# xander683/ConstructionScenePoseEstimation

Hardware: AMD Instinct MI355X
Metric: annotated frames/sec (RGB+seg+2D kpts) at 1920×1080, 1/2/4/8 MI355X (higher is better)
Workload: dtype f32

## Files before the change

constructionsceneposeestimation_amd/build.py:

```python
from __future__ import annotations

import os
import shutil
import subprocess
import sys

PKG = os.path.dirname(os.path.abspath(__file__))
ROOT = os.path.dirname(PKG)
LIB = os.path.join(PKG, "libcsg.so")
SOURCES = [os.path.join(PKG, "csrc", "csg_kernels.hip"), os.path.join(PKG, "csrc", "csg_encode.hip"),
           os.path.join(PKG, "csrc", "csg_crops.hip"), os.path.join(PKG, "csrc", "csg_spans.hip"),
           os.path.join(PKG, "csrc", "csg_amodal_spans.hip"), os.path.join(PKG, "csrc", "csg_api.cpp")]
DEPS = SOURCES + [os.path.join(PKG, "csrc", "csg_kernels.h"), os.path.join(PKG, "csrc", "csg_encode.h"),
                  os.path.join(PKG, "csrc", "csg_deflate.h"), os.path.join(PKG, "csrc", "csg_widen.h"),
                  os.path.join(PKG, "csrc", "csg_crops.h"), os.path.join(PKG, "csrc", "csg_spans.h"),
                  os.path.join(PKG, "csrc", "csg_amodal_spans.h"), os.path.join(PKG, "csrc", "csg_raster_math.h"),
                  os.path.join(PKG, "csrc", "csg_amodal_tri.inc"),
                  os.path.join(ROOT, "include", "csg_api.h")]
ARCH = os.environ.get("CSG_OFFLOAD_ARCH", "gfx950")
IO_LIB = os.path.join(PKG, "libcsgio.so")
IO_SOURCES = [os.path.join(PKG, "csrc", "csg_io.cpp")]
IO_DEPS = IO_SOURCES + [os.path.join(ROOT, "include", "csg_io.h"), os.path.join(PKG, "csrc", "csg_repr.h")]
IO_FLAGS = ["-O3", "-std=c++17", "-fPIC", "-shared", "-Wall", "-pthread"]
JSON_EXT = os.path.join(PKG, "_csgjson.so")
JSON_SOURCES = [os.path.join(PKG, "csrc", "csg_json.cpp"), os.path.join(PKG, "csrc", "csg_repr.h")]

FLAGS = ["-O3", "-std=c++17", "-fPIC", "-shared", "-ffp-contract=off", f"--offload-arch={ARCH}", "-Wall", "-pthread"]


def hipcc() -> str:
    for c in (os.environ.get("HIPCC"), "/opt/rocm/bin/hipcc", shutil.which("hipcc")):
        if c and os.path.exists(c):
            return c
    raise RuntimeError("hipcc not found (ROCm required to build libcsg.so)")


def needs_build(lib: str = LIB, deps=None) -> bool:
    deps = DEPS if deps is None else deps
    if not os.path.exists(lib):
        return True
    t = os.path.getmtime(lib)
    return any(os.path.getmtime(p) > t for p in deps)


def build(force: bool = False, verbose: bool = False) -> str:
    if force or needs_build():
        cmd = [hipcc(), *FLAGS, "-o", LIB + ".tmp", *SOURCES]
        if verbose:
            print(" ".join(cmd), file=sys.stderr)
        subprocess.run(cmd, check=True)
# ... 33 lines not shown
```

constructionsceneposeestimation_amd/csrc/csg_api.cpp:

```cpp
#include <hip/hip_runtime.h>
#include <stdint.h>
#include <stdlib.h>
#include <string.h>

#include <algorithm>
#include <cstddef>
#include <cmath>
#include <cstdarg>
#include <cstdio>
#include <memory>
#include <string>
#include <vector>

#include "../../include/csg_api.h"
#include "csg_amodal_spans.h"
#include "csg_crops.h"
#include "csg_encode.h"
#include "csg_kernels.h"
#include "csg_spans.h"
#include "csg_widen.h"

using namespace csg;

namespace {

template <class T>
struct DevBuf {
  T* p = nullptr;
  size_t n = 0;
  DevBuf() = default;
  DevBuf(const DevBuf&) = delete;
  DevBuf& operator=(const DevBuf&) = delete;
  ~DevBuf() { release(); }
  hipError_t alloc(size_t count) {
    if (count <= n && p) return hipSuccess;
    if (p) (void)hipFree(p);
    p = nullptr;
    n = 0;
    if (count == 0) return hipSuccess;
    hipError_t e = hipMalloc(reinterpret_cast<void**>(&p), count * sizeof(T));
    if (e == hipSuccess) n = count;
    return e;
  }
  void release() {
    if (p) (void)hipFree(p);
    p = nullptr;
    n = 0;
  }
};

constexpr uint32_t kAutoChainFrames = 0xFFFFFFFFu;

constexpr uint32_t kMaxSets = 65536;

struct HostTexture {
  std::vector<uint8_t> rgba;
  uint32_t w = 0, h = 0;
  bool present = false;
};

}

struct csg_ctx {
  csg_config cfg{};
  std::string err;
  hipStream_t stream = nullptr;
  uint32_t tiles_x = 0, tiles_y = 0, n_tiles = 0;

  bool have_scene = false;
  uint32_t n_inst = 0, n_meshes = 0, n_materials = 0;
  uint64_t n_tris_total = 0;
  DevBuf<float> tri_pos, tri_uv;
  DevBuf<InstDesc> inst;
  std::vector<MatDesc> h_mats;
  std::vector<MatDesc> h_set_mats;
  std::vector<MeshDesc> h_meshes;
  DevBuf<Chunk> chunks;
  uint32_t n_chunks = 0;
  uint32_t uid_shift = kUidShift;
  std::vector<HostTexture> textures;
  bool tex_dirty = true;
  DevBuf<uint8_t> texels;
  DevBuf<uint32_t> aquad;
  DevBuf<uint32_t> acls;
  std::vector<int> acls_thr;
  DevBuf<TexDesc> texd;
  LightDev light{{0.26f, 0.29f, 0.34f}, {0.78f, 0.78f, 0.78f}, {0.7071f, 0.f, 0.7071f},
                 191u | (217u << 8) | (255u << 16)};
  std::vector<LightDev> dr_light;
  std::vector<uint8_t> dr_light_valid;
  std::vector<int32_t> dr_tex;
  bool dr_dirty = true;
  DevBuf<LightDev> lights;
  DevBuf<MatDesc> set_mats;
  uint32_t n_table_sets = 0;
  std::vector<float> h_models;
  std::vector<uint8_t> set_valid;
  DevBuf<float> models;
  bool models_dirty = true;
  uint32_t n_kp = 0;
  std::vector<float> h_kp;
  std::vector<uint8_t> kp_valid;
  DevBuf<float> kp;
  bool kp_dirty = true;
  uint32_t n_lab = 1;
// ... 158 lines not shown
    const double g = (x >= 1.0 / 8 && x < 3.0 / 8) ? 4 * x - 0.5 : (x >= 3.0 / 8 && x < 5.0 / 8) ? 1.0
                     : (x >= 5.0 / 8 && x < 7.0 / 8) ? -4 * x + 3.5 : 0.0;
    const double b = (x < 1.0 / 8) ? 4 * x + 0.5 : (x >= 1.0 / 8 && x < 3.0 / 8) ? 1.0
                     : (x >= 3.0 / 8 && x < 5.0 / 8) ? -4 * x + 2.5 : 0.0;
    const double ch[3] = {r, g, b};
    uint32_t v = 0;
    for (int c = 0; c < 3; ++c) {
      const float p = (float)ch[c] * 255.0f;
      const long q = std::lrint(p);
      v |= (uint32_t)std::min(255L, std::max(0L, q)) << (8 * c);
    }
    lut[k] = v;
  }
}

extern "C" {

int csg_abi_version(void) { return CSG_ABI_VERSION; }

const char* csg_last_error(const csg_ctx* ctx) { return ctx ? ctx->err.c_str() : "null context"; }

int csg_create(const csg_config* cfg, csg_ctx** out) {
  if (!cfg || !out) return CSG_ERR_INVALID;
  *out = nullptr;
  if (cfg->width == 0 || cfg->height == 0 || cfg->width > 256u * kTileW || cfg->height > 512u * kTileH ||
      cfg->max_frames == 0 ||
      !(cfg->near_clip >= 0x1p-126f) || !(cfg->far_clip > cfg->near_clip) || !(cfg->far_clip <= 0x1p126f))
    return CSG_ERR_INVALID;
  csg_ctx* c = new csg_ctx();
  c->cfg = *cfg;
  if (const char* d = getenv("CSG_DEBUG")) c->dbg = (uint32_t)strtoul(d, nullptr, 0);
  if (const char* v = getenv("CSG_NARROW_IDS")) c->narrow_ids = atoi(v) != 0;
  if (const char* v = getenv("CSG_SPLIT_PAGEABLE")) c->split_pageable = atoi(v) != 0;
  c->chain_frames = cfg->frames_per_launch ? cfg->frames_per_launch : kAutoChainFrames;
  if (const char* v = getenv("CSG_CHAIN")) c->chain_frames = (uint32_t)std::max(1, atoi(v));
  c->chain_frames = std::min(c->chain_frames, cfg->max_frames);
  c->tiles_x = (cfg->width + kTileW - 1) / kTileW;
  c->tiles_y = (cfg->height + kTileH - 1) / kTileH;
  c->n_tiles = c->tiles_x * c->tiles_y;
  c->bin_blocks = kTileH >= 32 ? 32u : (c->n_tiles > 8192u ? 8u : 16u);
  if (const char* v = getenv("CSG_BINBLOCKS")) c->bin_blocks = std::max(1, std::min(1024, atoi(v)));
  hipError_t e = hipSetDevice(cfg->device);
  if (e == hipSuccess) e = hipStreamCreateWithFlags(&c->stream, hipStreamNonBlocking);
  c->ring.assign((size_t)csg_ctx::kRing * 5, nullptr);
  c->ring_frames.assign(csg_ctx::kRing, 0);
  for (size_t k = 0; k < c->ring.size() && e == hipSuccess; ++k) e = hipEventCreate(&c->ring[k]);
  for (uint32_t k = 0; k < csg_ctx::kStaging && e == hipSuccess; ++k)
    e = hipEventCreateWithFlags(&c->stage_ev[k], hipEventDisableTiming);
  if (e == hipSuccess) e = c->overflow.alloc(16);
  if (e == hipSuccess) e = hipMemset(c->overflow.p, 0, 16 * sizeof(uint32_t));
  if (e == hipSuccess) e = c->jet.alloc(256);
  if (e == hipSuccess) {
    uint32_t lut[256];
    jet_lut(lut);
    e = hipMemcpy(c->jet.p, lut, sizeof(lut), hipMemcpyHostToDevice);
  }
  c->ev = c->ring.data();
  if (e != hipSuccess) {
    c->err = hipGetErrorString(e);
    csg_destroy(c);
    return CSG_ERR_DEVICE;
  }
  *out = c;
  return CSG_OK;
}

void csg_destroy(csg_ctx* c) {
  if (!c) return;
  if (c->last_stream && c->last_stream != c->stream) (void)hipStreamSynchronize(c->last_stream);
  if (c->stream) (void)hipStreamSynchronize(c->stream);
  if (c->copy_stream) (void)hipStreamSynchronize(c->copy_stream);
  c->tri_pos.release(); c->tri_uv.release(); c->inst.release(); c->set_mats.release(); c->iset.release(); c->lights.release();
  c->chunks.release();
  c->texels.release();
  c->aquad.release();
  c->acls.release();
  c->texd.release(); c->models.release(); c->kp.release(); c->frames.release(); c->clip.release();
  c->pv.release(); c->recs.release(); c->rect.release(); c->rec_count.release(); c->tile_count.release();
  c->slab.release(); c->plan_need.release();
  c->tile_off.release(); c->bins.release(); c->bcount.release(); c->overflow.release(); c->o_rgb.release();
  c->o_inst.release(); c->o_depth.release(); c->o_kp_uv.release(); c->o_kp_vis.release(); c->o_stats.release();
  c->kp_w.release(); c->kp_pix.release(); c->kp_tiles.release();
  c->o_points.release(); c->o_normals.release(); c->cam.release(); c->fset.release();
  c->of.release(); c->o_objc.release();
  c->o_dvis.release(); c->o_drange.release(); c->o_cov.release(); c->drange.release(); c->jet.release();
  for (uint32_t k = 0; k < csg_ctx::kStaging; ++k) {
    if (c->h_stage[k]) (void)hipHostFree(c->h_stage[k]);
    if (c->stage_ev[k]) (void)hipEventDestroy(c->stage_ev[k]);
  }
  if (c->am_busy) (void)hipEventSynchronize(c->am_done);
  c->lab_off.release(); c->lab_chunks.release(); c->am_frames.release(); c->am_bits.release(); c->am_keys.release();
  for (uint32_t k = 0; k < csg_ctx::kStaging; ++k) {
    if (c->am_stage[k]) (void)hipHostFree(c->am_stage[k]);
    if (c->am_stage_ev[k]) (void)hipEventDestroy(c->am_stage_ev[k]);
  }
  c->as_planes.release(); c->as_touched.release(); c->as_cnt.release(); c->as_tables.release();
  if (c->as_stage) (void)hipHostFree(c->as_stage);
  if (c->as_stage_ev) (void)hipEventDestroy(c->as_stage_ev);
  if (c->am_done) (void)hipEventDestroy(c->am_done);
  if (c->ms_busy) (void)hipEventSynchronize(c->ms_done);
  c->ms_cnt.release();
  if (c->ms_done) (void)hipEventDestroy(c->ms_done);
  for (auto& e : c->ring)
    if (e) (void)hipEventDestroy(e);
  if (c->h_ids_n) (void)hipHostFree(c->h_ids_n);
// ... 108 lines not shown
  HIP_TRY(c, c->chunks.alloc(ch.size()));
  HIP_TRY(c, hipMemcpy(c->tri_pos.p, tri_pos.data(), tri_pos.size() * 4, hipMemcpyHostToDevice));
  HIP_TRY(c, hipMemcpy(c->tri_uv.p, tri_uv.data(), tri_uv.size() * 4, hipMemcpyHostToDevice));
  HIP_TRY(c, hipMemcpy(c->inst.p, idesc.data(), idesc.size() * sizeof(InstDesc), hipMemcpyHostToDevice));
  c->h_inst = idesc;
  {
    int32_t lo = -1, hi = -1;
    for (const InstDesc& d : idesc) { lo = std::min(lo, d.label); hi = std::max(hi, d.label); }
    c->ids_bytes = lo < -1 ? 4u : hi <= 254 ? 1u : hi <= 65534 ? 2u : 4u;
    c->n_lab = (uint32_t)std::max<int64_t>((int64_t)hi + 1, 1);
  }
  {
    std::vector<uint32_t> off((size_t)c->n_lab + 1, 0u), list;
    for (const Chunk& k : ch)
      if (idesc[k.inst].label >= 0) ++off[(size_t)idesc[k.inst].label + 1];
    uint32_t most = 0;
    for (uint32_t l = 0; l < c->n_lab; ++l) {
      most = std::max(most, off[l + 1]);
      off[l + 1] += off[l];
    }
    list.resize(std::max<size_t>(off[c->n_lab], 1), 0u);
    std::vector<uint32_t> at(off.begin(), off.end() - 1);
    for (size_t k = 0; k < ch.size(); ++k)
      if (idesc[ch[k].inst].label >= 0) list[at[(size_t)idesc[ch[k].inst].label]++] = (uint32_t)k;
    HIP_TRY(c, c->lab_off.alloc(off.size()));
    HIP_TRY(c, c->lab_chunks.alloc(list.size()));
    HIP_TRY(c, hipMemcpy(c->lab_off.p, off.data(), off.size() * 4, hipMemcpyHostToDevice));
    HIP_TRY(c, hipMemcpy(c->lab_chunks.p, list.data(), list.size() * 4, hipMemcpyHostToDevice));
    c->lab_max_chunks = most;
    c->h_lab_off = off;
    c->h_lab_chunks = list;
  }
  c->iset.release();
  HIP_TRY(c, hipMemcpy(c->chunks.p, ch.data(), ch.size() * sizeof(Chunk), hipMemcpyHostToDevice));
  c->n_inst = n_inst;
  c->n_meshes = n_meshes;
  c->n_materials = n_materials;
  c->h_mats = mats;
  c->h_meshes = md;
  c->n_chunks = (uint32_t)ch.size();
  c->n_tris_total = ntot;
  c->h_models = models;
  c->set_valid.assign(1, 1);
  c->models_dirty = true;
  c->dr_tex.clear();
  c->dr_dirty = true;
  c->h_kp.clear();
  c->kp_valid.clear();
  c->n_kp = 0;
  c->kp_dirty = true;
  c->h_of.clear();
  c->of_sets = 0;
  c->of_dirty = true;
  c->have_scene = true;
  c->work_frames = 0;
  c->rec_cap = 0;
  c->bin_cap = 0;
  return CSG_OK;
}

int csg_upload_texture(csg_ctx* c, uint32_t tex_id, const uint8_t* rgba8, uint32_t w, uint32_t h) {
  if (!c) return CSG_ERR_INVALID;
  if (!rgba8 || w == 0 || h == 0 || w > 16384 || h > 16384 || tex_id >= 4096)
    return c->fail(CSG_ERR_INVALID, "upload_texture: bad arguments");
  if (c->textures.size() <= tex_id) c->textures.resize(tex_id + 1);
  HostTexture& t = c->textures[tex_id];
// ... 104 lines not shown

static int build_alpha_classes(csg_ctx* c, const std::vector<TexDesc>& td, size_t total, bool tex_changed) {
  std::vector<int> thr(c->textures.size(), -1);
  for (const MatDesc& m : c->h_set_mats) {
    if (!m.alpha_test || m.texture < 0 || (size_t)m.texture >= thr.size()) continue;
    int& t = thr[m.texture];
    if (t == -1) t = (int)m.alpha_threshold;
    else if (t != (int)m.alpha_threshold) t = -2;
  }
  if (!tex_changed && c->acls.p && thr == c->acls_thr) return CSG_OK;
  c->acls_thr = thr;
  std::vector<uint32_t> cls((total + 15) / 16 + 1, 0xFFFFFFFFu);
  for (size_t k = 0; k < c->textures.size(); ++k) {
    const HostTexture& t = c->textures[k];
    if (!t.present || thr[k] < 0) continue;
    const uint32_t th = (uint32_t)thr[k];
    for (uint32_t y = 0; y < t.h; ++y)
      for (uint32_t x = 0; x < t.w; ++x) {
        const uint32_t x1 = x + 1 == t.w ? 0 : x + 1, y1 = y + 1 == t.h ? 0 : y + 1;
        auto a = [&](uint32_t xx, uint32_t yy) { return (uint32_t)t.rgba[((size_t)yy * t.w + xx) * 4 + 3]; };
        const uint32_t q[4] = {a(x, y), a(x1, y), a(x, y1), a(x1, y1)};
        const uint32_t mn = std::min(std::min(q[0], q[1]), std::min(q[2], q[3]));
        const uint32_t mx = std::max(std::max(q[0], q[1]), std::max(q[2], q[3]));
        const uint32_t cl = mx <= th ? 0u : mn > th ? 1u : 3u;
        const size_t i = (size_t)td[k].offset + (size_t)y * t.w + x;
        cls[i >> 4] = (cls[i >> 4] & ~(3u << (2 * (i & 15)))) | (cl << (2 * (i & 15)));
      }
  }
  HIP_TRY(c, c->acls.alloc(cls.size()));
  HIP_TRY(c, hipMemcpy(c->acls.p, cls.data(), cls.size() * 4, hipMemcpyHostToDevice));
  return CSG_OK;
}

static int sync_scene_state(csg_ctx* c) {
  const uint32_t n_sets = (uint32_t)c->set_valid.size();
  if (c->tex_dirty || c->dr_dirty || c->models_dirty || (c->kp_dirty && c->n_kp) || c->n_table_sets != n_sets) {
    const int rc = drain(c);
    if (rc) return rc;
    if (c->am_busy) HIP_TRY(c, hipEventSynchronize(c->am_done));
  }
  const bool tex_changed = c->tex_dirty;
  const bool iset_dirty = c->tex_dirty || c->dr_dirty || c->n_table_sets != n_sets || !c->iset.p;
  const bool cls_dirty = c->tex_dirty || c->dr_dirty || c->n_table_sets != n_sets || !c->acls.p;
  std::vector<TexDesc> td(c->textures.size());
  size_t total = 0;
  for (size_t k = 0; k < c->textures.size(); ++k) {
    td[k] = TexDesc{(uint32_t)total, c->textures[k].w, c->textures[k].h, 0};
    total += ((size_t)c->textures[k].w * c->textures[k].h + kTexAlign - 1) / kTexAlign * kTexAlign;
  }
  if (total / kTexAlign >= 0xFFFFFFu)
    return c->fail(CSG_ERR_LIMIT, "textures hold %zu texels; at most %u", total, 0xFFFFFFu * kTexAlign);
  if (c->tex_dirty) {
    HIP_TRY(c, c->texels.alloc(std::max<size_t>(total * 4, 4)));
    HIP_TRY(c, c->aquad.alloc(std::max<size_t>(total, 1)));
    HIP_TRY(c, c->texd.alloc(std::max<size_t>(td.size(), 1)));
    std::vector<uint32_t> quad;
    for (size_t k = 0; k < c->textures.size(); ++k)
      if (c->textures[k].present) {
        const HostTexture& t = c->textures[k];
        HIP_TRY(c, hipMemcpy(c->texels.p + (size_t)td[k].offset * 4, t.rgba.data(), t.rgba.size(),
                             hipMemcpyHostToDevice));
        quad.resize((size_t)t.w * t.h);
        for (uint32_t y = 0; y < t.h; ++y)
          for (uint32_t x = 0; x < t.w; ++x) {
            const uint32_t x1 = x + 1 == t.w ? 0 : x + 1, y1 = y + 1 == t.h ? 0 : y + 1;
            auto a = [&](uint32_t xx, uint32_t yy) { return (uint32_t)t.rgba[((size_t)yy * t.w + xx) * 4 + 3]; };
            quad[(size_t)y * t.w + x] = a(x, y) | (a(x1, y) << 8) | (a(x, y1) << 16) | (a(x1, y1) << 24);
          }
        HIP_TRY(c, hipMemcpy(c->aquad.p + td[k].offset, quad.data(), quad.size() * 4, hipMemcpyHostToDevice));
      }
    if (!td.empty()) HIP_TRY(c, hipMemcpy(c->texd.p, td.data(), td.size() * sizeof(TexDesc), hipMemcpyHostToDevice));
    c->tex_dirty = false;
  }
  if (c->dr_dirty || c->n_table_sets != n_sets) {
    std::vector<MatDesc> sm((size_t)n_sets * c->n_materials);
    std::vector<LightDev> sl(n_sets);
    for (uint32_t set = 0; set < n_sets; ++set) {
      sl[set] = (set < c->dr_light_valid.size() && c->dr_light_valid[set]) ? c->dr_light[set] : c->light;
      for (uint32_t m = 0; m < c->n_materials; ++m) {
        MatDesc d = c->h_mats[m];
        const size_t k = (size_t)set * c->n_materials + m;
        if (k < c->dr_tex.size() && c->dr_tex[k] != CSG_KEEP_TEXTURE) d.texture = c->dr_tex[k];
        sm[(size_t)set * c->n_materials + m] = d;
      }
    }
    HIP_TRY(c, c->set_mats.alloc(std::max<size_t>(sm.size(), 1)));
    HIP_TRY(c, c->lights.alloc(std::max<size_t>(sl.size(), 1)));
    c->h_set_mats = sm;
    if (!sm.empty()) HIP_TRY(c, hipMemcpy(c->set_mats.p, sm.data(), sm.size() * sizeof(MatDesc), hipMemcpyHostToDevice));
    if (!sl.empty()) HIP_TRY(c, hipMemcpy(c->lights.p, sl.data(), sl.size() * sizeof(LightDev), hipMemcpyHostToDevice));
    c->n_table_sets = n_sets;
    c->dr_dirty = false;
  }
  if (cls_dirty) {
    const int rc = build_alpha_classes(c, td, total, tex_changed);
    if (rc) return rc;
  }
  for (size_t k = 0; k < c->h_set_mats.size(); ++k) {
    const int t = c->h_set_mats[k].texture;
    if (t >= 0 && ((size_t)t >= c->textures.size() || !c->textures[t].present))
      return c->fail(CSG_ERR_INVALID, "material %u (set %u) references texture %d that was not uploaded",
                     (unsigned)(k % c->n_materials), (unsigned)(k / c->n_materials), t);
  }
  if (iset_dirty) {
    std::vector<InstSetDev> is((size_t)n_sets * c->n_inst);
    for (uint32_t set = 0; set < n_sets; ++set)
      for (uint32_t i = 0; i < c->n_inst; ++i) {
        const InstDesc& d = c->h_inst[i];
        const MatDesc& m = c->h_set_mats[(size_t)set * c->n_materials + d.material];
        InstSetDev e{};
        e.tex = (m.texture >= 0 && d.has_uv) ? m.texture : -1;
        e.base = (uint32_t)m.base[0] | ((uint32_t)m.base[1] << 8) | ((uint32_t)m.base[2] << 16);
        e.atex = kNoAlpha;
        if (m.alpha_test && m.texture >= 0) {
          const TexDesc& t = td[(size_t)m.texture];
          e.atex = t.offset;
          e.atex_wh = t.width | (t.height << 16);
          e.athr = m.alpha_threshold;
        }
        e.label = d.label;
        e.alpha_uv = (m.alpha_test && d.has_uv) ? 1u : 0u;
        is[(size_t)set * c->n_inst + i] = e;
      }
    HIP_TRY(c, c->iset.alloc(std::max<size_t>(is.size(), 1)));
    if (!is.empty()) HIP_TRY(c, hipMemcpy(c->iset.p, is.data(), is.size() * sizeof(InstSetDev), hipMemcpyHostToDevice));
  }
  if (c->models_dirty) {
    HIP_TRY(c, c->models.alloc(c->h_models.size()));
    HIP_TRY(c, hipMemcpy(c->models.p, c->h_models.data(), c->h_models.size() * 4, hipMemcpyHostToDevice));
    c->models_dirty = false;
  }
  if (c->kp_dirty && c->n_kp) {
    HIP_TRY(c, c->kp.alloc(c->h_kp.size()));
    HIP_TRY(c, hipMemcpy(c->kp.p, c->h_kp.data(), c->h_kp.size() * 4, hipMemcpyHostToDevice));
    c->kp_dirty = false;
  }
  return CSG_OK;
}

static int sync_object_frames(csg_ctx* c) {
  const uint32_t n_sets = (uint32_t)c->set_valid.size();
  if (!c->of_dirty && c->of_table_sets == n_sets && c->of.p) return CSG_OK;
  const int rc = drain(c);
  if (rc) return rc;
  if (c->am_busy) HIP_TRY(c, hipEventSynchronize(c->am_done));
  const size_t per = (size_t)c->n_lab * 12;
  std::vector<float> t((size_t)n_sets * per, 0.f);
  const size_t have = std::min<size_t>(c->of_sets, n_sets) * per;
  if (have) memcpy(t.data(), c->h_of.data(), have * sizeof(float));
  HIP_TRY(c, c->of.alloc(std::max<size_t>(t.size(), 12)));
  if (!t.empty()) HIP_TRY(c, hipMemcpy(c->of.p, t.data(), t.size() * 4, hipMemcpyHostToDevice));
  c->of_table_sets = n_sets;
  c->of_dirty = false;
  return CSG_OK;
// ... 48 lines not shown
                                       : (uint32_t)std::min<uint64_t>(3ull * c->rec_cap + 16ull * c->n_tiles,
                                                                      0x7FFFFFFCull);
  uint64_t rp, bp;
  target_pools(c, maxF, rp, bp);
  if (rp != c->rec_pool || bp != c->bin_pool) {
    c->recs.release(); c->rect.release(); c->bins.release();
  }
  HIP_TRY(c, c->frames.alloc(c->cfg.max_frames));
  for (uint32_t k = 0; k < csg_ctx::kStaging; ++k)
    if (!c->h_stage[k])
      HIP_TRY(c, hipHostMalloc(reinterpret_cast<void**>(&c->h_stage[k]), sizeof(FrameDev) * c->cfg.max_frames));
  HIP_TRY(c, c->fset.alloc(maxF));
  HIP_TRY(c, c->clip.alloc((size_t)maxF * c->n_inst * 12));
  HIP_TRY(c, c->pv.alloc((size_t)maxF * 12));
  HIP_TRY(c, c->cam.alloc((size_t)maxF * kCamFloats));
  c->rec_pool = c->bin_pool = 0;
  HIP_TRY(c, c->recs.alloc(rp));
  HIP_TRY(c, c->rect.alloc(rp));
  HIP_TRY(c, c->bins.alloc(bp));
  c->rec_pool = rp;
  c->bin_pool = bp;
  HIP_TRY(c, c->rec_count.alloc((size_t)maxF * kCounterStride));
  HIP_TRY(c, c->tile_count.alloc((size_t)maxF * c->n_tiles));
  HIP_TRY(c, c->tile_off.alloc((size_t)maxF * (c->n_tiles + 1)));
  HIP_TRY(c, c->bcount.alloc((size_t)maxF * c->bin_blocks * c->n_tiles));
  HIP_TRY(c, c->slab.alloc(maxF));
  HIP_TRY(c, c->plan_need.alloc(2));
  c->work_frames = maxF;
  return CSG_OK;
}

static SceneDev scene_dev(const csg_ctx* c) {
  SceneDev s{};
  s.tri_pos = c->tri_pos.p; s.tri_uv = c->tri_uv.p; s.inst = c->inst.p;
  s.texd = c->texd.p; s.texels = c->texels.p; s.aquad = c->aquad.p; s.acls = c->acls.p; s.n_inst = c->n_inst;
  s.W = c->cfg.width; s.H = c->cfg.height;
  s.tiles_x = c->tiles_x; s.tiles_y = c->tiles_y; s.n_tiles = c->n_tiles;
  s.near_clip = c->cfg.near_clip; s.far_clip = c->cfg.far_clip;
  s.inv_near = 1.0f / c->cfg.near_clip; s.inv_far = 1.0f / c->cfg.far_clip;
  s.dbg = c->dbg;
  s.uid_shift = c->uid_shift;
  s.rect_ys = c->tiles_y > 256u ? 1u : 0u;
  return s;
}

static bool host_pinned(const void* p) {
  hipPointerAttribute_t a{};
  if (hipPointerGetAttributes(&a, p) != hipSuccess) {
    (void)hipGetLastError();
    return false;
  }
  return a.type == hipMemoryTypeHost;
}

struct WidenChain {
  const void* src;
  uint32_t bytes;
  int32_t* dst;
  size_t n;
  std::shared_ptr<WidenLatch> latch;
};
static void widen_submit_cb(void* p) {
  std::unique_ptr<WidenChain> w(static_cast<WidenChain*>(p));
  WidenPool::get().submit(w->src, w->bytes, w->dst, w->n, w->latch);
}
static void widen_wait_cb(void* p) {
  std::unique_ptr<std::shared_ptr<WidenLatch>> l(static_cast<std::shared_ptr<WidenLatch>*>(p));
// ... 1310 lines not shown
```

constructionsceneposeestimation_amd/csrc/csg_kernels.h:

```cpp
#pragma once
#include <hip/hip_runtime.h>
#include <stdint.h>

namespace csg {

#ifndef CSG_TILE_W
#define CSG_TILE_W 32
#endif
#ifndef CSG_TILE_H
#define CSG_TILE_H 16
#endif
constexpr int kTileW = CSG_TILE_W;
constexpr int kTileH = CSG_TILE_H;
constexpr int kTilePix = kTileW * kTileH;
constexpr int kRasterBlock = kTilePix / 4;
static_assert((kTileW == 16 || kTileW == 32 || kTileW == 64) && (kTileH == 16 || kTileH == 32) &&
                  kRasterBlock >= 64 && kRasterBlock <= 256,
              "tile shapes: width 16/32/64, height 16/32, 64..256 threads");
constexpr int kBlock = 256;
constexpr uint32_t kUidShift = 20;
constexpr uint32_t kMaxInstances = 1u << (32 - kUidShift);
constexpr uint32_t kMaxTrisPerMesh = 1u << kUidShift;
#ifndef CSG_LDS_LABELS
#define CSG_LDS_LABELS ((CSG_TILE_W) * (CSG_TILE_H) >= 1024 ? 256 : 64)
#endif
constexpr int kMaxLdsLabels = CSG_LDS_LABELS;
constexpr int kCovSlots = 32;
constexpr uint32_t kCovUnknown = 0x80000000u;
constexpr uint32_t kCounterStride = 64;
constexpr uint32_t kNoAlpha = 0xFFFFFFFFu;
constexpr uint32_t kCamFloats = 16;

struct MeshDesc { uint32_t vbase, tbase, ntris, uvbase, has_uv, material; };
struct InstDesc { uint32_t tbase, material, has_uv; int32_t label; };
struct MatDesc { uint8_t base[4]; int32_t texture; uint32_t alpha_test, alpha_threshold; };
struct InstSetDev {
  int32_t tex;
  uint32_t base;
  uint32_t atex;
  uint32_t atex_wh;
  uint32_t athr;
  int32_t label;
  uint32_t alpha_uv;
  uint32_t pad;
};
static_assert(sizeof(InstSetDev) == 32, "InstSetDev layout");
struct TexDesc { uint32_t offset, width, height, pad; };
struct LightDev { float ambient[3], sun[3], sun_dir[3]; uint32_t sky; };
struct Chunk {
  uint32_t inst, start, count;
  uint32_t soup;
  float lo[3], hi[3];
  uint32_t pad2[2];
};
static_assert(sizeof(Chunk) == 48, "Chunk layout");

struct __attribute__((aligned(16))) Rec {
  int32_t x[3], y[3];
  uint16_t px0, py0, px1, py1;
  uint32_t uid;
  uint32_t atex;
  float D0, D1;
  float UV[3][2];
  float D2;
  uint32_t atex_wh;
};
static_assert(sizeof(Rec) == 80, "Rec layout");
constexpr int kRecGroups = 5;
constexpr uint32_t kTexAlign = 16;
__host__ __device__ inline uint32_t rec_atex(uint32_t offset, uint32_t thr) { return (offset / kTexAlign) | (thr << 24); }

struct FrameDev {
  float view[16];
  float proj[16];
  uint32_t xform_set;
  uint32_t frame_id;
  uint32_t records_hint;
  uint32_t bins_hint;
};

struct Slab {
  uint64_t rec_base, bin_base;
  uint32_t rec_cap, bin_cap;
  uint32_t pad[2];
};
static_assert(sizeof(Slab) == 32, "Slab layout");

struct SceneDev {
  const float* tri_pos;
  const float* tri_uv;
  const InstDesc* inst;
  const TexDesc* texd;
  const uint8_t* texels;
  const uint32_t* aquad;
  const uint32_t* acls;
  uint32_t n_inst;
  uint32_t W, H, tiles_x, tiles_y, n_tiles;
  float near_clip, far_clip;
  float inv_near, inv_far;
  uint32_t dbg;
  uint32_t uid_shift;
  uint32_t rect_ys;
};

constexpr uint32_t kOvRecords = 1u;
constexpr uint32_t kOvBins = 2u;
constexpr uint32_t kOvBadSet = 4u;
constexpr uint32_t kOvBadKpSet = 8u;

struct BatchDev {
  const FrameDev* frames;
  uint32_t* fset;
  uint32_t n_sets;
  uint32_t n_kp_sets;
  const float* models;
  const MatDesc* mats;
  const InstSetDev* iset;
  const LightDev* lights;
  uint32_t n_mat;
  float* clip;
  float* pv;
  Rec* recs;
  uint32_t* rect;
// ... 86 lines not shown
```

constructionsceneposeestimation_amd/csrc/csg_kernels.hip:

```cpp
#include <math.h>

#include <algorithm>

#include <type_traits>

#include "csg_crops.h"
#include "csg_kernels.h"
#include "csg_raster_math.h"

namespace csg {

#ifndef CSG_ABLATION
#define CSG_ABLATION 0
#endif
#define DBG(d) (CSG_ABLATION ? (d) : 0u)

constexpr uint64_t kEmptyKey = ~0ull;

__device__ __forceinline__ uint32_t fbits(float f) { return __float_as_uint(f); }

template <int Ctrl, int RowMask, int BankMask>
__device__ __forceinline__ uint32_t dpp_add(uint32_t v) {
  return v + (uint32_t)__builtin_amdgcn_update_dpp(0, (int)v, Ctrl, RowMask, BankMask, false);
}
// ... 84 lines not shown
    }
    frame_camera(fr.view, fr.proj, b.cam + (size_t)f * kCamFloats);
  }
}

__device__ __forceinline__ uint32_t rec_tile_rect(const SubRec& r, uint32_t ys) {
  const uint32_t px0 = r.g1.z & 0xFFFFu, py0 = r.g1.z >> 16, px1 = r.g1.w & 0xFFFFu, py1 = r.g1.w >> 16;
  return (px0 / kTileW) | (((py0 / kTileH) >> ys) << 8) | ((px1 / kTileW) << 16) | (((py1 / kTileH) >> ys) << 24);
}

__device__ __forceinline__ uint32_t rect_ty0(uint32_t rc, uint32_t ys) { return ((rc >> 8) & 255u) << ys; }
__device__ __forceinline__ uint32_t rect_ty1(uint32_t rc, uint32_t ys, uint32_t tiles_y) {
  return min((((rc >> 24) + 1u) << ys) - 1u, tiles_y - 1u);
}

__device__ __forceinline__ uint32_t rect_area(uint32_t rc, uint32_t ys, uint32_t tiles_y) {
  const uint32_t tx0 = rc & 255u, tx1 = (rc >> 16) & 255u;
  return (tx1 - tx0 + 1) * (rect_ty1(rc, ys, tiles_y) - rect_ty0(rc, ys) + 1);
}


__device__ __forceinline__ uint32_t rect_tile(uint32_t rc, uint32_t q, uint32_t tiles_x, uint32_t ys) {
  const uint32_t tx0 = rc & 255u, ty0 = rect_ty0(rc, ys), tx1 = (rc >> 16) & 255u;
  const uint32_t w = tx1 - tx0 + 1;
  const uint32_t r = small_div(q, w);
  return __umul24(ty0 + r, tiles_x) + tx0 + (q - __umul24(r, w));
}

typedef uint32_t v4u32 __attribute__((ext_vector_type(4)));

__device__ __forceinline__ void setup_chunk(const SceneDev& s, const BatchDev& b, const Chunk& ch, uint32_t f,
                                            int tid, int lane, uint4* sw);

__global__ __launch_bounds__(256) void k_setup(SceneDev s, BatchDev b, const Chunk* __restrict__ chunks,
                                               uint32_t n_chunks) {
  const uint32_t f = blockIdx.x, chunk = blockIdx.y + blockIdx.z * gridDim.y;
  if (chunk >= n_chunks) return;
  const int tid = threadIdx.x, lane = tid & 63;
  if (DBG(b.dbg) & 32u) return;
  const Chunk& ch = chunks[chunk];
  {
    const CullOut o = corner_out(s, ch, b.clip + ((size_t)f * s.n_inst + ch.inst) * 12, lane & 7);
    const uint64_t m8 = 0xFFull;
    const bool cull = ((__ballot(o.n) & m8) == m8) || ((__ballot(o.f) & m8) == m8) ||
                      ((__ballot(o.l) & m8) == m8) || ((__ballot(o.r) & m8) == m8) ||
                      ((__ballot(o.t) & m8) == m8) || ((__ballot(o.b) & m8) == m8);
    if (cull || (DBG(b.dbg) & 64u)) return;
  }
  static_assert(16 * kRecGroups <= 2 * 64, "two chunk stores per lane");
  __shared__ uint4 tstage[kBlock / 64][16 * kRecGroups];
  setup_chunk(s, b, ch, f, tid, lane, tstage[tid >> 6]);
}

__device__ __forceinline__ void setup_chunk(const SceneDev& s, const BatchDev& b, const Chunk& ch, uint32_t f,
                                            int tid, int lane, uint4* sw) {
  const uint32_t i = ch.inst;
  const float* Cm = b.clip + ((size_t)f * s.n_inst + i) * 12;

  SubRec r0, r1;
  uint4 c2 = make_uint4(0u, 0u, 0u, 0u), c3 = c2, c4 = c2;
  int nrec = 0;
  if ((uint32_t)tid < ch.count) {
    const uint32_t g = ch.soup + tid;
    Cv3 v[3];
    float c[12];
#pragma unroll
    for (int k = 0; k < 12; ++k) c[k] = Cm[k];
    const float* tp = s.tri_pos + (size_t)g * 9;
// ... 50 lines not shown
      auto emit_tri_r = [&](const Cv3& a, float ra, const Cv3& bb, float rb, const Cv3& cc, float rc) {
        float su[3], sv[3];
        su[0] = a.x * ra; sv[0] = a.y * ra;
        su[1] = bb.x * rb; sv[1] = bb.y * rb;
        su[2] = cc.x * rc; sv[2] = cc.y * rc;
        SubRec rr;
        if (make_rec(s, su, sv, rr)) {
          if (nrec == 0) r0 = rr; else r1 = rr;
          ++nrec;
        }
      };
      auto emit_tri = [&](const Cv3& a, const Cv3& bb, const Cv3& cc) {
        emit_tri_r(a, rcp_w(a.w), bb, rcp_w(bb.w), cc, rcp_w(cc.w));
      };
      if (nq >= 3) emit_tri(q0, q1, q2);
      if (nq >= 4) emit_tri(q0, q2, q3);
      if (nrec > 0) {
        Hom h;
        hom_setup(v, h);
        if (!h.ok) {
          nrec = 0;
        } else {
          const InstSetDev is = b.iset[(size_t)b.fset[f] * s.n_inst + i];
          const uint32_t atex = is.atex == kNoAlpha ? kNoAlpha : rec_atex(is.atex, is.athr), atex_wh = is.atex_wh;
          if (is.atex != kNoAlpha && is.athr >= 255u) nrec = 0;
          float D[3], U[3] = {0.0f, 0.0f, 0.0f}, V[3] = {0.0f, 0.0f, 0.0f};
          depth_plane(h.A, h.B, h.C, h.invdet, D);
          if (is.alpha_uv) {
            const float* tu = s.tri_uv + (size_t)g * 6;
            float uv[6];
#pragma unroll
            for (int k = 0; k < 6; ++k) uv[k] = tu[k];
            uv_planes(h.A, h.B, h.C, h.invdet, uv, U, V);
          }
          c2 = make_uint4(uid, atex, __float_as_uint(D[0]), __float_as_uint(D[1]));
          c3 = make_uint4(__float_as_uint(U[0]), __float_as_uint(V[0]), __float_as_uint(U[1]), __float_as_uint(V[1]));
          c4 = make_uint4(__float_as_uint(U[2]), __float_as_uint(V[2]), __float_as_uint(D[2]), atex_wh);
        }
      }
    }
  }
  const uint64_t b1 = __ballot(nrec >= 1), b2 = __ballot(nrec >= 2);
  const uint64_t lt = (lane == 0) ? 0ull : (~0ull >> (64 - lane));
  const uint32_t mine = (uint32_t)(__popcll(b1 & lt) + __popcll(b2 & lt));
  const uint32_t wtot = (uint32_t)(__popcll(b1) + __popcll(b2));
  uint32_t wbase = 0;
  if (lane == 0 && wtot) wbase = atomicAdd(&b.rec_count[f * kCounterStride], wtot);
  wbase = __shfl(wbase, 0, 64);
  if (DBG(b.dbg) & 128u) {
    if (nrec == 3 && b.inst) b.inst[0] = r0.g0.x + r1.g0.x + c2.x + c3.x + c4.x;
    return;
  }
  const uint64_t rbase = b.slab[f].rec_base;
  const uint32_t rcap = b.slab[f].rec_cap;
  if (lane == 0 && wbase + wtot > rcap) atomicOr(b.overflow, 1u);
  uint4* dst = reinterpret_cast<uint4*>(b.recs + rbase);
  const size_t lim = (size_t)rcap * kRecGroups;
  auto put = [&](uint32_t at, const SubRec& r) {
    uint4* o = sw + at * kRecGroups;
    o[0] = r.g0;
    o[1] = r.g1;
    o[2] = c2;
    o[3] = c3;
    o[4] = c4;
  };
  for (uint32_t p0 = 0; p0 < wtot; p0 += 16) {
// ... 1800 lines not shown
```

constructionsceneposeestimation_amd/csrc/csg_raster_math.h:

```cpp
#pragma once
#include <math.h>

#include "csg_kernels.h"

namespace csg {

constexpr int kSmallCover = 4;
constexpr float kGuardPx = 1048576.0f;

typedef float f32x2 __attribute__((ext_vector_type(2)));

__device__ __forceinline__ float dot4(const float* r, float x, float y, float z) {
  return ((r[0] * x + r[1] * y) + r[2] * z) + r[3];
}

__device__ __forceinline__ void mat4_mul(const float* a, const float* b, float* c) {
#pragma unroll
  for (int i = 0; i < 4; ++i)
#pragma unroll
    for (int j = 0; j < 4; ++j)
      c[i * 4 + j] = ((a[i * 4 + 0] * b[0 * 4 + j] + a[i * 4 + 1] * b[1 * 4 + j]) + a[i * 4 + 2] * b[2 * 4 + j]) +
                     a[i * 4 + 3] * b[3 * 4 + j];
}

// ... 173 lines not shown
    for (int k = 1; k < N; ++k) {
      nwm += __any(nw >= k) ? 1 : 0;
      nhm += __any(nh >= k) ? 1 : 0;
    }
    int32_t er[3] = {e0[0], e0[1], e0[2]};
#pragma unroll
    for (int j = 0; j < N; ++j) {
      if (j > nhm) break;
      int32_t ec[3] = {er[0], er[1], er[2]};
#pragma unroll
      for (int i = 0; i < N; ++i) {
        if (i > nwm) break;
        const bool in = i <= nw && j <= nh && (ec[0] | ec[1] | ec[2]) >= 0;
        cols |= in ? 1u << i : 0u;
        rows |= in ? 1u << j : 0u;
#pragma unroll
        for (int e = 0; e < 3; ++e) ec[e] += sx[e];
      }
#pragma unroll
      for (int e = 0; e < 3; ++e) er[e] += sy[e];
    }
    if (!cols) return false;
    px1 = px0 + 31 - __clz(cols);
    px0 += __ffs(cols) - 1;
    py1 = py0 + 31 - __clz(rows);
    py0 += __ffs(rows) - 1;
  }
  r.g0 = make_uint4((uint32_t)x[0], (uint32_t)x[1], (uint32_t)x[2], (uint32_t)y[0]);
  r.g1 = make_uint4((uint32_t)y[1], (uint32_t)y[2], (uint32_t)px0 | ((uint32_t)py0 << 16),
                    (uint32_t)px1 | ((uint32_t)py1 << 16));
  return true;
}

__device__ __forceinline__ uint32_t small_div(uint32_t q, uint32_t w) {
  uint32_t d = (uint32_t)((float)q * __builtin_amdgcn_rcpf((float)w));
  const uint32_t p = __umul24(d, w);
  d = p > q ? d - 1u : (p + w <= q ? d + 1u : d);
  return d;
}

struct CullOut { bool n, f, l, r, t, b; };
__device__ __forceinline__ CullOut corner_out(const SceneDev& s, const Chunk& ch, const float* Cm, int c) {
  const float px = (c & 4) ? ch.hi[0] : ch.lo[0];
  const float py = (c & 2) ? ch.hi[1] : ch.lo[1];
  const float pz = (c & 1) ? ch.hi[2] : ch.lo[2];
  const float X = dot4(Cm + 0, px, py, pz), Y = dot4(Cm + 4, px, py, pz), Wc = dot4(Cm + 8, px, py, pz);
  const float tol = 1e-3f * (fabsf(X) + fabsf(Y) + fabsf(Wc)) + 1e-3f;
  return CullOut{Wc < s.near_clip - tol, Wc > s.far_clip + tol, X < -tol, X > (float)s.W * Wc + tol * (float)s.W,
                 Y < -tol, Y > (float)s.H * Wc + tol * (float)s.H};
}

__device__ __forceinline__ float rcp_w(float w) { return w <= 0x1p126f ? rcp_ieee(w) : 1.0f / w; }

constexpr uint32_t kAmSerial = 16;
constexpr uint32_t kAmQueue = 64;
constexpr int32_t kAmPast = 0x7FFFFFFF;

struct AmTri {
  int32_t x[3], y[3];
  float D[3], U[3], V[3];
  uint32_t atex, wh, thr;
  uint32_t i0, ni, j0, nj;
};

template <bool kKey>
__device__ __forceinline__ bool amodal_hit(const SceneDev& s, const AmTri& t, int32_t px, int32_t py, uint32_t& key) {
// ... 22 lines not shown
```

Baseline: 24250.

## Trim alpha-tested triangle screen boxes using precomputed opaque texel UV bounds

Precomputes on the host, per alpha-tested triangle, a conservative UV bounding box of texels that pass the alpha threshold, and uploads it to the device. During setup, fully-inside triangles with a valid error guard shrink their pixel bounding box to the opaque region, or are dropped entirely when no texel passes. This is meant to reduce raster and coverage work for foliage/fence-like cutout geometry, at the cost of host preprocessing, an extra per-triangle load, and more setup arithmetic. It also forces k_setup to 8 waves per EU.

```diff
diff --git a/constructionsceneposeestimation_amd/build.py b/constructionsceneposeestimation_amd/build.py
--- a/constructionsceneposeestimation_amd/build.py
+++ b/constructionsceneposeestimation_amd/build.py
@@ -16,6 +16,7 @@
                   os.path.join(PKG, "csrc", "csg_crops.h"), os.path.join(PKG, "csrc", "csg_spans.h"),
                   os.path.join(PKG, "csrc", "csg_amodal_spans.h"), os.path.join(PKG, "csrc", "csg_raster_math.h"),
                   os.path.join(PKG, "csrc", "csg_amodal_tri.inc"),
+                  os.path.join(PKG, "csrc", "csg_alpha_box.h"),
                   os.path.join(ROOT, "include", "csg_api.h")]
 ARCH = os.environ.get("CSG_OFFLOAD_ARCH", "gfx950")
 IO_LIB = os.path.join(PKG, "libcsgio.so")
diff --git a/constructionsceneposeestimation_amd/csrc/csg_alpha_box.h b/constructionsceneposeestimation_amd/csrc/csg_alpha_box.h
--- /dev/null
+++ b/constructionsceneposeestimation_amd/csrc/csg_alpha_box.h
@@ -0,0 +1,120 @@
+#pragma once
+#include <algorithm>
+#include <cmath>
+#include <cstdint>
+#include <vector>
+
+namespace csg {
+
+constexpr double kAlphaScanGuard = 2.0;
+constexpr double kAlphaBoxMargin = 0.5;
+constexpr double kAlphaMaxTexel = 4194304.0;
+
+struct AlphaScan {
+  uint32_t w = 0, h = 0;
+  std::vector<int32_t> next, prev;
+};
+
+inline void alpha_scan_build(const uint8_t* rgba, uint32_t w, uint32_t h, uint32_t thr, AlphaScan& s) {
+  s.w = w;
+  s.h = h;
+  s.next.assign((size_t)w * h, (int32_t)w);
+  s.prev.assign((size_t)w * h, -1);
+  auto a = [&](uint32_t x, uint32_t y) { return (uint32_t)rgba[((size_t)y * w + x) * 4 + 3]; };
+  for (uint32_t y = 0; y < h; ++y) {
+    const uint32_t y1 = y + 1 == h ? 0 : y + 1;
+    int32_t* nx = &s.next[(size_t)y * w];
+    int32_t* pv = &s.prev[(size_t)y * w];
+    int32_t last = -1;
+    for (uint32_t x = 0; x < w; ++x) {
+      const uint32_t x1 = x + 1 == w ? 0 : x + 1;
+      const uint32_t mx = std::max(std::max(a(x, y), a(x1, y)), std::max(a(x, y1), a(x1, y1)));
+      if (mx > thr) last = (int32_t)x;
+      pv[x] = last;
+    }
+    int32_t nxt = (int32_t)w;
+    for (uint32_t x = w; x-- > 0;) {
+      if (pv[x] == (int32_t)x) nxt = (int32_t)x;
+      nx[x] = nxt;
+    }
+  }
+}
+
+inline void alpha_box_full(float* box) {
+  box[0] = box[2] = -INFINITY;
+  box[1] = box[3] = INFINITY;
+}
+inline void alpha_box_empty(float* box) {
+  box[0] = box[2] = INFINITY;
+  box[1] = box[3] = -INFINITY;
+}
+
+inline float alpha_round_down(double x) {
+  float f = (float)x;
+  return (double)f > x ? std::nextafterf(f, -INFINITY) : f;
+}
+inline float alpha_round_up(double x) {
+  float f = (float)x;
+  return (double)f < x ? std::nextafterf(f, INFINITY) : f;
+}
+
+inline void alpha_tri_box(const AlphaScan& s, const float* uv, float* box) {
+  alpha_box_full(box);
+  const double G = kAlphaScanGuard;
+  const int64_t tw = s.w, th = s.h;
+  if (tw == 0 || th == 0) return;
+  double tx[3], ty[3];
+  for (int k = 0; k < 3; ++k) {
+    tx[k] = (double)uv[2 * k] * (double)tw - 0.5;
+    ty[k] = (1.0 - (double)uv[2 * k + 1]) * (double)th - 0.5;
+    if (!(std::fabs(tx[k]) < kAlphaMaxTexel) || !(std::fabs(ty[k]) < kAlphaMaxTexel)) return;
+  }
+  const double xmin = std::min(tx[0], std::min(tx[1], tx[2])), xmax = std::max(tx[0], std::max(tx[1], tx[2]));
+  const double ymin = std::min(ty[0], std::min(ty[1], ty[2])), ymax = std::max(ty[0], std::max(ty[1], ty[2]));
+  const int64_t bx0 = (int64_t)std::floor(xmin - G), bx1 = (int64_t)std::floor(xmax + G);
+  const int64_t j0 = (int64_t)std::floor(ymin - G), j1 = (int64_t)std::floor(ymax + G);
+  if (bx1 - bx0 + 1 > tw || j1 - j0 + 1 > th) return;
+  bool any = false;
+  int64_t qx0 = 0, qx1 = 0, qy0 = 0, qy1 = 0;
+  for (int64_t j = j0; j <= j1; ++j) {
+    const double lo = (double)j - G, hi = (double)j + 1.0 + G;
+    double ex0 = INFINITY, ex1 = -INFINITY;
+    for (int k = 0; k < 3; ++k) {
+      const int n = k == 2 ? 0 : k + 1;
+      if (ty[k] >= lo && ty[k] <= hi) { ex0 = std::min(ex0, tx[k]); ex1 = std::max(ex1, tx[k]); }
+      for (const double yb : {lo, hi}) {
+        if ((ty[k] < yb && ty[n] > yb) || (ty[k] > yb && ty[n] < yb)) {
+          const double x = tx[k] + (tx[n] - tx[k]) * ((yb - ty[k]) / (ty[n] - ty[k]));
+          ex0 = std::min(ex0, x);
+          ex1 = std::max(ex1, x);
+        }
+      }
+    }
+    if (!(ex0 <= ex1)) continue;
+    const int64_t a = std::max(bx0, (int64_t)std::floor(ex0 - G)), b = std::min(bx1, (int64_t)std::floor(ex1 + G));
+    if (a > b) continue;
+    const int64_t jr = ((j % th) + th) % th, ar = ((a % tw) + tw) % tw;
+    const int32_t* nx = &s.next[(size_t)jr * tw];
+    const int32_t* pv = &s.prev[(size_t)jr * tw];
+    const int64_t len = b - a, e1 = std::min<int64_t>(ar + len, tw - 1);
+    int64_t first = INT64_MAX, last = INT64_MIN;
+    if (nx[ar] <= e1) { first = a + (nx[ar] - ar); last = a + (pv[e1] - ar); }
+    if (ar + len >= tw) {
+      const int64_t e2 = ar + len - tw, off = a + (tw - ar);
+      if (nx[0] <= e2) { first = std::min(first, off + nx[0]); last = std::max(last, off + pv[e2]); }
+    }
+    if (first > last) continue;
+    if (!any) { qx0 = first; qx1 = last; qy0 = qy1 = j; any = true; }
+    qx0 = std::min(qx0, first);
+    qx1 = std::max(qx1, last);
+    qy1 = j;
+  }
+  if (!any) { alpha_box_empty(box); return; }
+  const double M = kAlphaBoxMargin;
+  box[0] = alpha_round_down(((double)qx0 + 0.5 - M) / (double)tw);
+  box[1] = alpha_round_up(((double)qx1 + 1.5 + M) / (double)tw);
+  box[2] = alpha_round_down(1.0 - ((double)qy1 + 1.5 + M) / (double)th);
+  box[3] = alpha_round_up(1.0 - ((double)qy0 + 0.5 - M) / (double)th);
+}
+
+}
diff --git a/constructionsceneposeestimation_amd/csrc/csg_api.cpp b/constructionsceneposeestimation_amd/csrc/csg_api.cpp
--- a/constructionsceneposeestimation_amd/csrc/csg_api.cpp
+++ b/constructionsceneposeestimation_amd/csrc/csg_api.cpp
@@ -8,11 +8,14 @@
 #include <cmath>
 #include <cstdarg>
 #include <cstdio>
+#include <map>
 #include <memory>
 #include <string>
+#include <utility>
 #include <vector>
 
 #include "../../include/csg_api.h"
+#include "csg_alpha_box.h"
 #include "csg_amodal_spans.h"
 #include "csg_crops.h"
 #include "csg_encode.h"
@@ -71,6 +74,10 @@
   uint32_t n_inst = 0, n_meshes = 0, n_materials = 0;
   uint64_t n_tris_total = 0;
   DevBuf<float> tri_pos, tri_uv;
+  DevBuf<float> abox;
+  std::vector<float> h_tri_uv;
+  std::vector<int32_t> h_abox_tex;
+  bool alpha_trim = true;
   DevBuf<InstDesc> inst;
   std::vector<MatDesc> h_mats;
   std::vector<MatDesc> h_set_mats;
@@ -295,6 +302,7 @@
   if (const char* d = getenv("CSG_DEBUG")) c->dbg = (uint32_t)strtoul(d, nullptr, 0);
   if (const char* v = getenv("CSG_NARROW_IDS")) c->narrow_ids = atoi(v) != 0;
   if (const char* v = getenv("CSG_SPLIT_PAGEABLE")) c->split_pageable = atoi(v) != 0;
+  if (const char* v = getenv("CSG_ALPHA_TRIM")) c->alpha_trim = atoi(v) != 0;
   c->chain_frames = cfg->frames_per_launch ? cfg->frames_per_launch : kAutoChainFrames;
   if (const char* v = getenv("CSG_CHAIN")) c->chain_frames = (uint32_t)std::max(1, atoi(v));
   c->chain_frames = std::min(c->chain_frames, cfg->max_frames);
@@ -333,7 +341,7 @@
   if (c->last_stream && c->last_stream != c->stream) (void)hipStreamSynchronize(c->last_stream);
   if (c->stream) (void)hipStreamSynchronize(c->stream);
   if (c->copy_stream) (void)hipStreamSynchronize(c->copy_stream);
-  c->tri_pos.release(); c->tri_uv.release(); c->inst.release(); c->set_mats.release(); c->iset.release(); c->lights.release();
+  c->tri_pos.release(); c->tri_uv.release(); c->abox.release(); c->inst.release(); c->set_mats.release(); c->iset.release(); c->lights.release();
   c->chunks.release();
   c->texels.release();
   c->aquad.release();
@@ -508,6 +516,8 @@
     c->h_lab_chunks = list;
   }
   c->iset.release();
+  c->abox.release();
+  c->h_tri_uv = tri_uv;
   HIP_TRY(c, hipMemcpy(c->chunks.p, ch.data(), ch.size() * sizeof(Chunk), hipMemcpyHostToDevice));
   c->n_inst = n_inst;
   c->n_meshes = n_meshes;
@@ -678,6 +688,42 @@
   return CSG_OK;
 }
 
+static int build_alpha_boxes(csg_ctx* c) {
+  const size_t n_soup = c->h_tri_uv.size() / 6;
+  std::vector<float> box(std::max<size_t>(n_soup, 1) * 4);
+  for (size_t g = 0; g < box.size() / 4; ++g) alpha_box_full(&box[g * 4]);
+  c->h_abox_tex.assign(c->h_meshes.size(), -1);
+  std::map<std::pair<int, uint32_t>, AlphaScan> scans;
+  for (size_t m = 0; m < c->h_meshes.size() && c->alpha_trim; ++m) {
+    const MeshDesc& d = c->h_meshes[m];
+    const MatDesc& mat = c->h_mats[d.material];
+    if (!d.has_uv || !mat.alpha_test || mat.texture < 0 || (size_t)mat.texture >= c->textures.size() ||
+        !c->textures[mat.texture].present || mat.alpha_threshold >= 255u)
+      continue;
+    const HostTexture& t = c->textures[mat.texture];
+    AlphaScan& sc = scans[{mat.texture, mat.alpha_threshold}];
+    if (sc.w == 0) alpha_scan_build(t.rgba.data(), t.w, t.h, mat.alpha_threshold, sc);
+    for (uint32_t k = 0; k < d.ntris; ++k) {
+      const size_t g = (size_t)d.tbase + k;
+      alpha_tri_box(sc, &c->h_tri_uv[g * 6], &box[g * 4]);
+    }
+    c->h_abox_tex[m] = mat.texture;
+  }
+  HIP_TRY(c, c->abox.alloc(box.size()));
+  HIP_TRY(c, hipMemcpy(c->abox.p, box.data(), box.size() * 4, hipMemcpyHostToDevice));
+  return CSG_OK;
+}
+
+static bool same_alpha(const csg_ctx* c, int a, int b) {
+  if (a == b) return true;
+  const HostTexture& x = c->textures[a];
+  const HostTexture& y = c->textures[b];
+  if (x.w != y.w || x.h != y.h) return false;
+  for (size_t k = 3; k < x.rgba.size(); k += 4)
+    if (x.rgba[k] != y.rgba[k]) return false;
+  return true;
+}
+
 static int sync_scene_state(csg_ctx* c) {
   const uint32_t n_sets = (uint32_t)c->set_valid.size();
   if (c->tex_dirty || c->dr_dirty || c->models_dirty || (c->kp_dirty && c->n_kp) || c->n_table_sets != n_sets) {
@@ -688,6 +734,7 @@
   const bool tex_changed = c->tex_dirty;
   const bool iset_dirty = c->tex_dirty || c->dr_dirty || c->n_table_sets != n_sets || !c->iset.p;
   const bool cls_dirty = c->tex_dirty || c->dr_dirty || c->n_table_sets != n_sets || !c->acls.p;
+  const bool box_dirty = c->tex_dirty || !c->abox.p;
   std::vector<TexDesc> td(c->textures.size());
   size_t total = 0;
   for (size_t k = 0; k < c->textures.size(); ++k) {
@@ -748,8 +795,21 @@
       return c->fail(CSG_ERR_INVALID, "material %u (set %u) references texture %d that was not uploaded",
                      (unsigned)(k % c->n_materials), (unsigned)(k / c->n_materials), t);
   }
-  if (iset_dirty) {
+  if (box_dirty) {
+    const int rc = build_alpha_boxes(c);
+    if (rc) return rc;
+  }
+  if (iset_dirty || box_dirty) {
     std::vector<InstSetDev> is((size_t)n_sets * c->n_inst);
+    std::vector<int32_t> inst_mesh(c->n_inst, -1);
+    for (uint32_t i = 0; i < c->n_inst; ++i)
+      for (size_t m = 0; m < c->h_meshes.size(); ++m)
+        if (c->h_meshes[m].tbase == c->h_inst[i].tbase && c->h_meshes[m].material == c->h_inst[i].material &&
+            c->h_abox_tex[m] >= 0) {
+          inst_mesh[i] = (int32_t)m;
+          break;
+        }
+    std::map<std::pair<int, int>, bool> same;
     for (uint32_t set = 0; set < n_sets; ++set)
       for (uint32_t i = 0; i < c->n_inst; ++i) {
         const InstDesc& d = c->h_inst[i];
@@ -766,6 +826,13 @@
         }
         e.label = d.label;
         e.alpha_uv = (m.alpha_test && d.has_uv) ? 1u : 0u;
+        if (c->alpha_trim && e.alpha_uv && e.atex != kNoAlpha && inst_mesh[i] >= 0 &&
+            m.alpha_threshold == c->h_mats[d.material].alpha_threshold) {
+          const std::pair<int, int> key{c->h_abox_tex[inst_mesh[i]], m.texture};
+          auto it = same.find(key);
+          if (it == same.end()) it = same.emplace(key, same_alpha(c, key.first, key.second)).first;
+          e.trim = it->second ? 1u : 0u;
+        }
         is[(size_t)set * c->n_inst + i] = e;
       }
     HIP_TRY(c, c->iset.alloc(std::max<size_t>(is.size(), 1)));
@@ -880,7 +947,8 @@
 
 static SceneDev scene_dev(const csg_ctx* c) {
   SceneDev s{};
-  s.tri_pos = c->tri_pos.p; s.tri_uv = c->tri_uv.p; s.inst = c->inst.p;
+  s.tri_pos = c->tri_pos.p; s.tri_uv = c->tri_uv.p; s.tri_abox = reinterpret_cast<const float4*>(c->abox.p);
+  s.inst = c->inst.p;
   s.texd = c->texd.p; s.texels = c->texels.p; s.aquad = c->aquad.p; s.acls = c->acls.p; s.n_inst = c->n_inst;
   s.W = c->cfg.width; s.H = c->cfg.height;
   s.tiles_x = c->tiles_x; s.tiles_y = c->tiles_y; s.n_tiles = c->n_tiles;
diff --git a/constructionsceneposeestimation_amd/csrc/csg_kernels.h b/constructionsceneposeestimation_amd/csrc/csg_kernels.h
--- a/constructionsceneposeestimation_amd/csrc/csg_kernels.h
+++ b/constructionsceneposeestimation_amd/csrc/csg_kernels.h
@@ -42,7 +42,7 @@
   uint32_t athr;
   int32_t label;
   uint32_t alpha_uv;
-  uint32_t pad;
+  uint32_t trim;
 };
 static_assert(sizeof(InstSetDev) == 32, "InstSetDev layout");
 struct TexDesc { uint32_t offset, width, height, pad; };
@@ -89,6 +89,7 @@
 struct SceneDev {
   const float* tri_pos;
   const float* tri_uv;
+  const float4* tri_abox;
   const InstDesc* inst;
   const TexDesc* texd;
   const uint8_t* texels;
diff --git a/constructionsceneposeestimation_amd/csrc/csg_kernels.hip b/constructionsceneposeestimation_amd/csrc/csg_kernels.hip
--- a/constructionsceneposeestimation_amd/csrc/csg_kernels.hip
+++ b/constructionsceneposeestimation_amd/csrc/csg_kernels.hip
@@ -140,8 +140,8 @@
 __device__ __forceinline__ void setup_chunk(const SceneDev& s, const BatchDev& b, const Chunk& ch, uint32_t f,
                                             int tid, int lane, uint4* sw);
 
-__global__ __launch_bounds__(256) void k_setup(SceneDev s, BatchDev b, const Chunk* __restrict__ chunks,
-                                               uint32_t n_chunks) {
+__global__ __launch_bounds__(256) __attribute__((amdgpu_waves_per_eu(8, 8))) void k_setup(
+    SceneDev s, BatchDev b, const Chunk* __restrict__ chunks, uint32_t n_chunks) {
   const uint32_t f = blockIdx.x, chunk = blockIdx.y + blockIdx.z * gridDim.y;
   if (chunk >= n_chunks) return;
   const int tid = threadIdx.x, lane = tid & 63;
@@ -258,6 +258,23 @@
 #pragma unroll
             for (int k = 0; k < 6; ++k) uv[k] = tu[k];
             uv_planes(h.A, h.B, h.C, h.invdet, uv, U, V);
+            if (is.trim && nq == 3 && in0 && in1 && in2 && nrec == 1) {
+              const float4 bx = s.tri_abox[g];
+              const bool none = bx.x > bx.y;
+              const float B = none ? 0.0f : fmaxf(fmaxf(fabsf(bx.x), fabsf(bx.y)), fmaxf(fabsf(bx.z), fabsf(bx.w)));
+              float m;
+              if (B < INFINITY &&
+                  alpha_trim_guard(v, uv, U, V, D, (float)max(atex_wh & 0xFFFFu, atex_wh >> 16), B, m)) {
+                int px0 = (int)(r0.g1.z & 0xFFFFu), py0 = (int)(r0.g1.z >> 16);
+                int px1 = (int)(r0.g1.w & 0xFFFFu), py1 = (int)(r0.g1.w >> 16);
+                if (none || !alpha_trim_box(U, V, D, bx, m, px0, py0, px1, py1)) {
+                  nrec = 0;
+                } else {
+                  r0.g1.z = (uint32_t)px0 | ((uint32_t)py0 << 16);
+                  r0.g1.w = (uint32_t)px1 | ((uint32_t)py1 << 16);
+                }
+              }
+            }
           }
           c2 = make_uint4(uid, atex, __float_as_uint(D[0]), __float_as_uint(D[1]));
           c3 = make_uint4(__float_as_uint(U[0]), __float_as_uint(V[0]), __float_as_uint(U[1]), __float_as_uint(V[1]));
diff --git a/constructionsceneposeestimation_amd/csrc/csg_raster_math.h b/constructionsceneposeestimation_amd/csrc/csg_raster_math.h
--- a/constructionsceneposeestimation_amd/csrc/csg_raster_math.h
+++ b/constructionsceneposeestimation_amd/csrc/csg_raster_math.h
@@ -229,6 +229,89 @@
   return true;
 }
 
+__device__ __forceinline__ float rcp_w(float w);
+constexpr float kTrimEps = 0x1p-20f;
+#ifndef CSG_TRIM_PASSES
+#define CSG_TRIM_PASSES 2
+#endif
+constexpr int kTrimPasses = CSG_TRIM_PASSES;
+
+__device__ __forceinline__ bool alpha_trim_guard(const Cv3* v, const float* uv, const float* U, const float* V,
+                                                 const float* D, float T, float B, float& m) {
+  float su[3], sv[3], X = 0.0f, Y = 0.0f, umax = 0.0f;
+#pragma unroll
+  for (int k = 0; k < 3; ++k) {
+    const float r = rcp_w(v[k].w);
+    su[k] = v[k].x * r;
+    sv[k] = v[k].y * r;
+    X = fmaxf(X, fabsf(su[k]));
+    Y = fmaxf(Y, fabsf(sv[k]));
+    umax = fmaxf(umax, fmaxf(fabsf(uv[2 * k]), fabsf(uv[2 * k + 1])));
+  }
+  X += 1.0f;
+  Y += 1.0f;
+  umax += 2.0f;
+  const float Sd = (fabsf(D[0]) * X + fabsf(D[1]) * Y) + fabsf(D[2]);
+  const float S = fmaxf((fabsf(U[0]) * X + fabsf(U[1]) * Y) + fabsf(U[2]), (fabsf(V[0]) * X + fabsf(V[1]) * Y) + fabsf(V[2]));
+  const float dD = kTrimEps * Sd + (fabsf(D[0]) + fabsf(D[1])) * (1.0f / 256.0f);
+  const float dU = kTrimEps * S + fmaxf(fabsf(U[0]) + fabsf(U[1]), fabsf(V[0]) + fabsf(V[1])) * (1.0f / 256.0f);
+  float dmin = INFINITY, res = 0.0f;
+#pragma unroll
+  for (int k = 0; k < 3; ++k) {
+    const float Dk = plane_at(D[0], D[1], D[2], su[k], sv[k]);
+    const float Uk = plane_at(U[0], U[1], U[2], su[k], sv[k]), Vk = plane_at(V[0], V[1], V[2], su[k], sv[k]);
+    dmin = fminf(dmin, Dk);
+    res = fmaxf(res, fmaxf(fabsf(Uk - uv[2 * k] * Dk), fabsf(Vk - uv[2 * k + 1] * Dk)));
+  }
+  dmin -= dD;
+  if (!(dmin >= 0x1p-100f)) return false;
+  if (!(((res + dU) + umax * dD) * T <= dmin)) return false;
+  if (!(kTrimEps * T * ((S + umax * Sd) + (umax + 1.0f) * dmin) <= 0.25f * dmin)) return false;
+  m = kTrimEps * (S + B * Sd);
+  return m < INFINITY;
+}
+
+__device__ __forceinline__ void trim_axis(float a, float b, float c, float m, float o0, float o1, int& lo, int& hi) {
+  if (!(a != 0.0f) || lo > hi) return;
+  const float est = -((fmaxf(b * o0, b * o1) + c) + m) * __builtin_amdgcn_rcpf(a);
+  const float e = fminf(fmaxf(est - 0.5f, (float)lo - 1.0f), (float)hi + 1.0f);
+  auto gone = [&](int p) {
+    const float t = (float)p + 0.5f;
+    return fmaxf((a * t + b * o0) + c, (a * t + b * o1) + c) < -m;
+  };
+  if (a > 0.0f) {
+    int n = max((int)ceilf(e), lo);
+    if (n > lo && !gone(n - 1)) {
+      --n;
+      if (n > lo && !gone(n - 1)) n = lo;
+    }
+    lo = n;
+  } else {
+    int n = min((int)floorf(e), hi);
+    if (n < hi && !gone(n + 1)) {
+      ++n;
+      if (n < hi && !gone(n + 1)) n = hi;
+    }
+    hi = n;
+  }
+}
+
+__device__ __forceinline__ bool alpha_trim_box(const float* U, const float* V, const float* D, float4 bx, float m,
+                                               int& px0, int& py0, int& px1, int& py1) {
+#pragma nounroll
+  for (int pass = 0; pass < kTrimPasses; ++pass) {
+#pragma unroll
+    for (int k = 0; k < 4; ++k) {
+      const float* P = k < 2 ? U : V;
+      const float bd = k == 0 ? bx.x : k == 1 ? bx.y : k == 2 ? bx.z : bx.w, sg = (k & 1) ? -1.0f : 1.0f;
+      const float h0 = sg * (P[0] - bd * D[0]), h1 = sg * (P[1] - bd * D[1]), h2 = sg * (P[2] - bd * D[2]);
+      trim_axis(h0, h1, h2, m, (float)py0 + 0.5f, (float)py1 + 0.5f, px0, px1);
+      trim_axis(h1, h0, h2, m, (float)px0 + 0.5f, (float)px1 + 0.5f, py0, py1);
+    }
+  }
+  return px0 <= px1 && py0 <= py1;
+}
+
 __device__ __forceinline__ uint32_t small_div(uint32_t q, uint32_t w) {
   uint32_t d = (uint32_t)((float)q * __builtin_amdgcn_rcpf((float)w));
   const uint32_t p = __umul24(d, w);
```

After: 25630 (median of 6 runs). +5.7%, better.
